# mprib/caliscope

Hardware: NVIDIA H100
Metric: lm_iterations_per_sec (higher is better)
Workload: dtype f64

## Files before the change

caliscope_b200/csrc/cb_device.cuh:

```cuda
#pragma once
#include <cuda_runtime.h>
#include <stdint.h>

namespace cb {

constexpr int CT_R = 0;
constexpr int CT_T = 9;
constexpr int CT_JR = 12;
constexpr int CT_FX = 21;
constexpr int CT_FY = 22;
constexpr int CT_CX = 23;
constexpr int CT_CY = 24;
constexpr int CT_D = 25;
constexpr int CT_IFX0 = 30;
constexpr int CT_SX = 31;
constexpr int CT_SY = 32;
constexpr int CT_FYR = 33;
constexpr int CT_FLAGS = 34;
constexpr int CT_FX0 = 35;
constexpr int CT_SIZE = 36;
constexpr int CT_SMEM = 37;

constexpr double CB_EPS = 2.220446049250313e-16;

// ... 23 lines not shown
  asm volatile("mbarrier.arrive.expect_tx.shared::cta.b64 _, [%0], %1;" ::"r"(smem_u32(bar)), "r"(bytes) : "memory");
}
__device__ __forceinline__ void mbar_wait(unsigned long long* bar, uint32_t phase) {
  asm volatile(
      "{\n"
      ".reg .pred p;\n"
      "WAIT_%=:\n"
      "mbarrier.try_wait.parity.shared::cta.b64 p, [%0], %1;\n"
      "@p bra DONE_%=;\n"
      "bra WAIT_%=;\n"
      "DONE_%=:\n"
      "}\n" ::"r"(smem_u32(bar)),
      "r"(phase)
      : "memory");
}
__device__ __forceinline__ void mbar_arrive(unsigned long long* bar) {
  asm volatile("mbarrier.arrive.shared::cta.b64 _, [%0];" ::"r"(smem_u32(bar)) : "memory");
}
__device__ __forceinline__ void bulk_g2s(void* dst_smem, const void* src_gmem, uint32_t bytes, unsigned long long* bar) {
  asm volatile("cp.async.bulk.shared::cluster.global.mbarrier::complete_tx::bytes [%0], [%1], %2, [%3];" ::"r"(
                   smem_u32(dst_smem)),
               "l"(src_gmem), "r"(bytes), "r"(smem_u32(bar))
               : "memory");
}

__device__ __forceinline__ double warp_sum(double v) {
#pragma unroll
  for (int o = 16; o > 0; o >>= 1) v += __shfl_xor_sync(0xffffffffu, v, o);
  return v;
}
__device__ __forceinline__ double warp_max(double v) {
#pragma unroll
  for (int o = 16; o > 0; o >>= 1) v = fmax(v, __shfl_xor_sync(0xffffffffu, v, o));
  return v;
}

__device__ __forceinline__ void loss_eval(int loss, double z, double& r0, double& r1, double& r2) {
  switch (loss) {
    case 1: {
      double t = 1.0 + z, s = sqrt(t);
      r0 = 2.0 * (s - 1.0);
      r1 = 1.0 / s;
      r2 = -0.5 / (t * s);
    } break;
    case 2: {
      if (z <= 1.0) {
// ... 192 lines not shown
```

caliscope_b200/csrc/cb_engine.cu:

```cuda
#include <cuda_runtime.h>
#include <dlfcn.h>
#if defined(__x86_64__)
#include <emmintrin.h>
#endif
#include <nvtx3/nvToolsExt.h>

#include <algorithm>
#include <atomic>
#include <chrono>
#include <cmath>
#include <cstdio>
#include <cstdlib>
#include <cstring>
#include <condition_variable>
#include <cub/cub.cuh>
#include <deque>
#include <functional>
#include <map>
#include <memory>
#include <mutex>
#include <string>
#include <thread>
#include <vector>

// ... 388 lines not shown
  size_t pt_smem = 0, bs_smem = 0;
  std::vector<int> h_cam_off;
  std::vector<int> h_perm, h_slot;
  std::vector<int> h_iflags;
  bool order_auto = false, order_identity = true;
  int ncp = 0;
  int *d_cam_xoff = nullptr, *d_cam_slot = nullptr, *d_klist = nullptr;
  bool schur_sparse = false;
  double schur_flop_issued = 0.0;
  std::vector<void*> allocs;
  int* d_cam_flags = nullptr;
  double* d_cam_const = nullptr;
  double2 *d_cm_xy = nullptr, *d_pm_xy = nullptr;
  int *d_cm_pt = nullptr, *d_cm_orig = nullptr, *d_cam_start = nullptr;
  int *d_chunk_cam = nullptr, *d_chunk_begin = nullptr, *d_chunk_end = nullptr, *d_cam_chunk_start = nullptr;
  int *d_pt_start = nullptr, *d_pm_orig = nullptr, *d_pm_cam = nullptr, *d_pm_pt = nullptr;
  const int *d_obs_cam = nullptr, *d_obs_pt = nullptr;
  const double* d_obs_xy = nullptr;
  std::vector<int> h_cam_flags;
  std::vector<double> h_cam_const;
  int *d_tile_of = nullptr, *d_tile_slot_start = nullptr, *d_tile_slots = nullptr;
  cb::SyItem* d_items = nullptr;
  int n_items = 0, n_slots = 0;
  unsigned char* d_active = nullptr;
  double *d_lo = nullptr, *d_hi = nullptr;
  double *d_x = nullptr, *d_xc[2] = {nullptr, nullptr}, *d_xp4[2] = {nullptr, nullptr};
  double *d_camtab[2] = {nullptr, nullptr}, *d_Upk[2] = {nullptr, nullptr}, *d_gc[2] = {nullptr, nullptr},
         *d_costsum[2] = {nullptr, nullptr};
  double *d_partial = nullptr, *d_camcost = nullptr, *d_V6 = nullptr, *d_gp = nullptr, *d_Dp2 = nullptr,
         *d_Dc2 = nullptr, *d_Linv6 = nullptr, *d_tvec = nullptr, *d_Zt = nullptr, *d_part = nullptr,
         *d_tpart = nullptr, *d_red = nullptr, *d_Minv = nullptr, *d_dc = nullptr, *d_dp = nullptr,
         *d_bpart = nullptr, *d_sc = nullptr, *d_red2 = nullptr, *d_out2 = nullptr;
  unsigned long long* d_gmax = nullptr;
  unsigned int* d_counter = nullptr;
  cb::LmState* d_state = nullptr;
  cb::LmState* h_state = nullptr;
  cb::LmLogRow* d_log = nullptr;
  int log_cap = 4096;
  double* h_x = nullptr;
  cudaEvent_t ev0 = nullptr, ev1 = nullptr, ev2 = nullptr, ev3 = nullptr, ev_state[2] = {nullptr, nullptr};
  cudaEvent_t ev_pp[2][4] = {{nullptr, nullptr, nullptr, nullptr}, {nullptr, nullptr, nullptr, nullptr}};
  cudaStream_t cap_stream = nullptr;
  TrialGraph trial_graph;
  TrialGraph loop_graph;
  int pcg_cs = 1, pcg_rows = 0, pcg_mode = 2, pcg_cl = 1, pcg_npa = 0;
  bool direct_solve = false;
// ... 319 lines not shown
  const int loss = 0;
  const double fscale = 1.0;
  launch_resjac<P, 0>(p, p->d_state, flip, loss, fscale, nullptr, st);
  if (p->n_c)
    CB_LAUNCH((cb::constraint_eval_kernel<false>), p->n_cblk, cb::CC_THREADS, 0, st, (const cb::LmState*)p->d_state, flip,
              p->ct, p->c_xp(), loss, fscale, p->m_crs(), p->m_cdirw(), (double*)nullptr, p->d_camcost + p->n_cams);
  CB_LAUNCH((cb::trial_reduce_kernel<P>), p->n_cams + 1, 64, 0, st, p->d_state, mode, p->n_cams, p->d_cam_chunk_start,
            p->d_partial, p->m_Upk(), p->m_gc(), p->m_costsum(), p->d_camcost, p->n_cblk, p->d_bpart,
            p->pt_grid + p->n_comp, p->pt_grid + p->n_comp, p->d_red2, p->d_counter, p->d_sc, p->d_log);
  return CB_OK;
}

template <int P>
int build_system(CbBaProblem* p, const CbBaOptions* opt, cudaStream_t st, const cudaEvent_t* ev = nullptr, bool cov = false) {
  if (ev) CB_CUDA(cudaEventRecord(ev[0], st));
  if (cov) launch_pt_pass<P, true>(p, st);
  else launch_pt_pass<P>(p, st);
  if (ev) CB_CUDA(cudaEventRecord(ev[1], st));
  if (p->n_c)
    CB_LAUNCH((cb::comp_build_kernel<P>), p->n_comp, cb::CC_THREADS, p->comp_build_smem, st, (const cb::LmState*)p->d_state,
              p->ct, p->d_pt_start, p->d_pm_cam, p->d_V6, p->d_gp, p->d_Dp2, p->d_gpt, p->c_crs(), p->c_cdirw(), p->n_cams,
              p->d_compL, p->d_tvec, p->d_Zt, (size_t)p->LD, p->d_gmax);
  if (ev) CB_CUDA(cudaEventRecord(ev[2], st));
  CB_LAUNCH(cb::schur_syrk_kernel, p->n_items, cb::SY_THREADS, sizeof(cb::SyrkSmem), st, (const cb::LmState*)p->d_state,
            p->d_Zt, (size_t)p->LD, p->d_tvec, p->d_items, (const int*)p->d_klist, p->d_part, p->d_tpart);
  if (ev) CB_CUDA(cudaEventRecord(ev[3], st));
  const size_t nfin = (size_t)p->nP * p->nP + p->nP + 1;
  const int rank = sharded(opt) ? std::min(std::max(opt->rank, 0), p->red_slots - 1) : 0;
  if (opt && opt->peer_group) {
    CbPeerGroup* g = (CbPeerGroup*)opt->peer_group;
    int nb = 0;
    CB_CUDA(cudaOccupancyMaxActiveBlocksPerMultiprocessor(&nb, cb::schur_finalize_peer_kernel<P>, cb::PEER_THREADS, 0));
    const int grid = std::max(1, std::min(nb, 2)) * p->num_sms;
    const cb::LmState* sd = p->d_state;
    int nP = p->nP, n_blk = p->n_blk, red_slots = p->red_slots, rk = rank;
    cb::CPtr2 upk = p->c_Upk(), gc = p->c_gc(), cs = p->c_costsum();
    const double* gmax = (const double*)p->d_gmax;
    void* args[] = {&sd, &nP, &n_blk, &p->d_tile_of, &p->d_tile_slot_start, &p->d_tile_slots, &p->d_part, &p->d_tpart,
                    &upk, &gc, &cs, &gmax, &red_slots, &rk, &g->tab, &p->d_red};
    CB_CUDA(cudaLaunchCooperativeKernel((const void*)cb::schur_finalize_peer_kernel<P>, dim3(grid), dim3(cb::PEER_THREADS),
                                        args, 0, st));
    g_launches.fetch_add(1);
  } else {
    CB_LAUNCH((cb::schur_finalize_kernel<P>), cdiv((long long)std::max<size_t>(nfin, p->red_slots), 256), 256, 0, st,
              (const cb::LmState*)p->d_state, p->nP, p->n_blk, p->d_tile_of, p->d_tile_slot_start, p->d_tile_slots,
              p->d_part, p->d_tpart, p->c_Upk(), p->c_gc(), p->c_costsum(), (const double*)p->d_gmax, p->red_slots, rank,
              p->d_red);
    if (sharded(opt)) CB_TRY(do_allreduce(opt, p->d_red, (long long)p->red_len(), st));
// ... 530 lines not shown
  switch (what) {
    case 0: return p->schur_sparse ? 1.0 : 0.0;
    case 1: return p->schur_flop_issued;
    case 2: return p->direct_solve ? 1.0 : 0.0;
    case 3: return (double)p->n_items;
    case 4: case 5: case 6: return (double)p->cov_ms[what - 4];
    case 7: return (double)p->pt_lanes;
    case 8: return p->n_dups ? 1.0 : 0.0;
    case 9: return (double)p->cam_in_smem;
    case 10: return p->direct_solve ? 0.0 : (double)p->pcg_mode;
    case 11: return (double)p->pcg_cs;
    case 12: return p->pcg_mode == 2 ? (double)p->pcg_cl : 0.0;
    case 13: return p->order_identity ? 0.0 : 1.0;
    default: return -1.0;
  }
}

static int build_schur_items(CbBaProblem* p, cudaStream_t st) {
  const int nb = p->n_blk;
  std::vector<int> tof((size_t)nb * nb, -1);
  int nt = 0;
  for (int I = 0; I < nb; ++I)
    for (int J = I; J < nb; ++J) tof[(size_t)I * nb + J] = nt++;
  const double w_pair = 1.31;
  const double w_single = 1.04;

  std::vector<long long> pair_koff, pair_cnt;
  bool sparse = false;
  int want_sparse = -1;
  if (const char* ev = std::getenv("CB_SY_SPARSE")) want_sparse = std::atoi(ev);
  if (nb >= 2 && nb <= 64 && p->n_pts > 0 && want_sparse != 0) {
    unsigned long long* d_mask;
    CB_TRY(dalloc(&d_mask, (size_t)p->n_pts));
    ScopedFree sf; sf.dev.push_back(d_mask);
    CB_LAUNCH(cb::pt_tile_mask_kernel, cdiv(p->n_pts, 256), 256, 0, st, p->d_pt_start, p->d_pm_cam, p->n_pts, p->P, d_mask);
    if (p->n_comp)
      CB_LAUNCH(cb::comp_tile_mask_kernel, cdiv(p->n_comp, 256), 256, 0, st, p->ct.comp_pt_start, p->ct.comp_pts, p->n_comp,
                d_mask);
    unsigned long long* d_cnt;
    CB_TRY(dalloc(&d_cnt, (size_t)nt));
    sf.dev.push_back(d_cnt);
    CB_CUDA(cudaMemsetAsync(d_cnt, 0, sizeof(unsigned long long) * nt, st));
    CB_LAUNCH(cb::tile_pair_count_kernel, cdiv(p->n_pts, 256), 256, sizeof(unsigned) * nt, st, d_mask, p->n_pts, nb, d_cnt);
    std::vector<unsigned long long> cnt_u((size_t)nt);
    CB_CUDA(cudaMemcpyAsync(cnt_u.data(), d_cnt, sizeof(unsigned long long) * nt, cudaMemcpyDeviceToHost, st));
    CB_CUDA(cudaStreamSynchronize(st));
    std::vector<long long> cnt(cnt_u.begin(), cnt_u.end());
    double listed = 0.0, dense = 0.0;
    for (int I = 0; I < nb; ++I)
      for (int J = I; J < nb; ++J) {
        const double w = (I == J) ? w_single : 1.0;
        listed += w * (double)cnt[tof[(size_t)I * nb + J]];
        dense += w * (double)p->n_pts;
      }
    sparse = want_sparse == 1 || listed < 0.7 * dense;
    if (sparse) {
      const int zero_row = p->K_pad;
      std::vector<long long> pair_start((size_t)nt + 1, 0), koff_h((size_t)nt, -1);
      long long klen = 0;
      for (int t = 0; t < nt; ++t) {
        pair_start[(size_t)t + 1] = pair_start[(size_t)t] + cnt[(size_t)t];
        if (cnt[(size_t)t] == 0) continue;
        koff_h[(size_t)t] = klen;
        klen += cdiv(3 * cnt[(size_t)t], (long long)cb::SY_KC) * cb::SY_KC;
      }
      const long long n_inc = pair_start[(size_t)nt];
      if (klen > 0x7fffffffLL || n_inc > 0x7fffffffLL) { g_last_error = "Schur row lists exceed 2^31 entries"; return CB_E_UNSUPPORTED; }
      pair_koff.assign(koff_h.begin(), koff_h.end());
      pair_cnt.assign(cnt.begin(), cnt.end());
      int *d_ninc = nullptr, *d_incoff = nullptr;
      unsigned long long *d_keys = nullptr, *d_keys_s = nullptr;
      long long *d_pair_start = nullptr, *d_koff = nullptr;
      CB_TRY(dalloc(&d_ninc, (size_t)p->n_pts + 1)); sf.dev.push_back(d_ninc);
      CB_TRY(dalloc(&d_incoff, (size_t)p->n_pts + 1)); sf.dev.push_back(d_incoff);
// ... 23 lines not shown
      CB_LAUNCH(cb::klist_expand_kernel, cdiv(n_inc, 256), 256, 0, st, (const unsigned long long*)d_keys_s, n_inc, p->n_pts,
                (const long long*)d_pair_start, (const long long*)d_koff, p->d_klist);
      CB_CUDA(cudaStreamSynchronize(st));
    }
  }
  p->schur_sparse = sparse;

  struct Group { int kind, I, J; double w; int chunks; int koff; };
  std::vector<Group> groups;
  if (!sparse) {
    for (int I = 0; I < nb; ++I)
      for (int J = I + 1; J < nb; ++J) groups.push_back({0, I, J, 1.0, p->k_chunks, -1});
    for (int I = 0; I < nb; I += 2) {
      if (I + 1 < nb) groups.push_back({1, I, I + 1, w_pair, p->k_chunks, -1});
      else groups.push_back({1, I, -1, w_single, p->k_chunks, -1});
    }
  } else {
    for (int I = 0; I < nb; ++I)
      for (int J = I; J < nb; ++J) {
        const int t = tof[(size_t)I * nb + J];
        if (pair_cnt[(size_t)t] == 0) continue;
        const int koff = (int)pair_koff[(size_t)t];
        const int chunks = (int)cdiv(3 * pair_cnt[(size_t)t], (long long)cb::SY_KC);
        if (I == J) groups.push_back({1, I, -1, w_single, chunks, koff});
        else groups.push_back({0, I, J, 1.0, chunks, koff});
      }
  }
  double W = 0.0;
  for (auto& g : groups) W += g.w * g.chunks;
  p->schur_flop_issued = 0.0;
  for (auto& g : groups) {
    const double cols2 = g.kind == 0 ? 96.0 * 96.0 : (g.J >= 0 ? 2.0 : 1.0) * 42.0 * 16.0 * 8.0;
    p->schur_flop_issued += 2.0 * cols2 * (double)g.chunks * cb::SY_KC;
  }
  std::vector<cb::SyItem> items;
  std::vector<std::vector<int>> slots_of(nt);
  int slot = 0;
  constexpr int SY_MIN_CHUNKS = 8;
  auto cap_of = [&](const Group& g) { return std::max(1, g.chunks / SY_MIN_CHUNKS); };
  std::vector<int> n_of(groups.size(), 1);
  {
    int used = 0;
    for (size_t gi = 0; gi < groups.size(); ++gi) {
      const Group& g = groups[gi];
      int n = (int)std::floor(p->num_sms * (g.w * g.chunks) / std::max(W, 1.0));
      n_of[gi] = std::max(1, std::min(n, cap_of(g)));
      used += n_of[gi];
// ... 301 lines not shown
  for (int c = 0; c < p->n_cams; ++c)
    for (int a = 0; a < ((p->h_iflags[c] & CB_CAM_FREE_INTRINSICS) ? 9 : 6); ++a) act[(size_t)c * p->P + a] = 1;
  CB_TRY(palloc(p, &p->d_active, p->nP));
  CB_CUDA(cudaMemcpyAsync(p->d_active, act.data(), p->nP, cudaMemcpyHostToDevice, st));
  CB_CUDA(cudaStreamSynchronize(st));
  CB_TRY(palloc(p, &p->d_lo, p->nP)); CB_TRY(palloc(p, &p->d_hi, p->nP));

  const int NACC = (p->P == 6) ? 28 : 55, NU = (p->P == 6) ? 21 : 45;
  const size_t npts = (size_t)std::max(p->n_pts, 1);
  CB_TRY(palloc(p, &p->d_x, (size_t)p->n_params + 1));
  for (int k = 0; k < 2; ++k) {
    CB_TRY(palloc(p, &p->d_xc[k], p->nP)); CB_TRY(palloc(p, &p->d_xp4[k], 4 * npts));
    CB_TRY(palloc(p, &p->d_camtab[k], (size_t)p->n_cams * cb::CT_SIZE));
    CB_TRY(palloc(p, &p->d_Upk[k], (size_t)p->n_cams * NU)); CB_TRY(palloc(p, &p->d_gc[k], p->nP));
    CB_TRY(palloc(p, &p->d_costsum[k], 4));
  }
  CB_TRY(palloc(p, &p->d_partial, (size_t)std::max(p->n_chunks, 1) * NACC + p->n_cblk));
  CB_TRY(palloc(p, &p->d_camcost, (size_t)p->n_cams + p->n_cblk));
  CB_TRY(palloc(p, &p->d_gpt, 3 * npts));
  CB_TRY(palloc(p, &p->d_V6, 6 * npts)); CB_TRY(palloc(p, &p->d_gp, 3 * npts)); CB_TRY(palloc(p, &p->d_Dp2, 3 * npts));
  CB_TRY(palloc(p, &p->d_Dc2, p->nP)); CB_TRY(palloc(p, &p->d_Linv6, 6 * npts));
  CB_TRY(palloc(p, &p->d_tvec, (size_t)p->K_pad + cb::SY_KC));
  CB_TRY(palloc(p, &p->d_Zt, ((size_t)p->K_pad + cb::SY_KC) * p->LD));
  CB_TRY(palloc(p, &p->d_part, (size_t)p->n_slots * cb::SY_TILE * cb::SY_TILE));
  CB_TRY(palloc(p, &p->d_tpart, (size_t)p->n_slots * cb::SY_TILE));
  CB_TRY(palloc(p, &p->d_red, p->red_len()));
  CB_TRY(palloc(p, &p->d_Minv, (size_t)p->n_cams * p->P * p->P));
  CB_TRY(palloc(p, &p->d_dc, p->nP)); CB_TRY(palloc(p, &p->d_dp, 3 * npts));
  CB_TRY(palloc(p, &p->d_bpart, 3 * ((size_t)p->pt_grid + p->n_comp)));
  CB_TRY(palloc(p, &p->d_sc, cb::SC_COUNT)); CB_TRY(palloc(p, &p->d_red2, 8));
  CB_TRY(palloc(p, &p->d_gmax, 2));
  CB_TRY(palloc(p, &p->d_counter, 4));
  CB_TRY(palloc(p, &p->d_state, 1));
  CB_TRY(palloc(p, &p->d_log, (size_t)p->log_cap));
  CB_TRY(palloc(p, &p->d_out2, 2 * (size_t)std::max(n, 1)));
  CB_CUDA(cudaMemsetAsync(p->d_Zt, 0, sizeof(double) * ((size_t)p->K_pad + cb::SY_KC) * p->LD, st));
  CB_CUDA(cudaMemsetAsync(p->d_tvec, 0, sizeof(double) * ((size_t)p->K_pad + cb::SY_KC), st));
  CB_CUDA(cudaMemsetAsync(p->d_tpart, 0, sizeof(double) * (size_t)p->n_slots * cb::SY_TILE, st));
  CB_CUDA(cudaMemsetAsync(p->d_part, 0, sizeof(double) * (size_t)p->n_slots * cb::SY_TILE * cb::SY_TILE, st));
  CB_CUDA(cudaMemsetAsync(p->d_red2, 0, sizeof(double) * 8, st));
  CB_CUDA(cudaMemsetAsync(p->d_Linv6, 0, sizeof(double) * 6 * npts, st));
  CB_TRY(cached_malloc_host((void**)&p->h_state, sizeof(cb::LmState) * 4));
  CB_TRY(cached_malloc_host((void**)&p->h_x, sizeof(double) * ((size_t)p->n_params + 1)));
  for (cudaEvent_t* e : {&p->ev0, &p->ev1, &p->ev2, &p->ev3, &p->ev_pp[0][0], &p->ev_pp[0][1], &p->ev_pp[0][2], &p->ev_pp[0][3],
                         &p->ev_pp[1][0], &p->ev_pp[1][1], &p->ev_pp[1][2], &p->ev_pp[1][3]})
    CB_CUDA(cudaEventCreate(e));
// ... 1824 lines not shown
```

caliscope_b200/csrc/cb_kernels.cuh:

```cuda
#pragma once
#include <cooperative_groups.h>

#include "cb_device.cuh"

namespace cb {
namespace cg = cooperative_groups;

constexpr int RJ_THREADS = 128;
constexpr int RJ_CHUNK = 2048;
constexpr int PT_WARPS = 8;
constexpr int SY_TILE = 96;
constexpr int SY_KC = 32;
constexpr int SY_STAGES = 4;
constexpr int SY_CONSUMER_WARPS = 8;
constexpr int SY_THREADS = 32 * (SY_CONSUMER_WARPS + 1);
constexpr int PCG_THREADS = 512;

template <int P>
struct RowT {
  static constexpr int NU = P * (P + 1) / 2;
  static constexpr int NACC = NU + P + 1;
};

enum {
// ... 245 lines not shown
  const double e00 = V6[0] + lam * d0, e01 = V6[1], e02 = V6[2], e11 = V6[3] + lam * d1, e12 = V6[4],
               e22 = V6[5] + lam * d2;
  bool ok = e00 > 0.0;
  const double i00 = rsqrt(ok ? e00 : 1.0);
  const double l10 = e01 * i00, l20 = e02 * i00;
  const double t11 = e11 - l10 * l10;
  ok = ok && t11 > 0.0;
  const double i11 = rsqrt(ok ? t11 : 1.0);
  const double l21 = (e12 - l20 * l10) * i11;
  const double t22 = e22 - l20 * l20 - l21 * l21;
  ok = ok && t22 > 0.0;
  const double i22 = rsqrt(ok ? t22 : 1.0);
  const double i10 = -l10 * i00 * i11;
  const double i21 = -l21 * i11 * i22;
  const double i20 = -(l20 * i00 + l21 * i10) * i22;
  if (ok) {
    Li[0] = i00; Li[1] = i10; Li[2] = i11; Li[3] = i20; Li[4] = i21; Li[5] = i22;
  } else {
    Li[0] = Li[1] = Li[2] = Li[3] = Li[4] = Li[5] = 0.0;
  }
}

constexpr int SY_LDS = SY_TILE + 4;

struct SyrkSmem {
  double A[SY_STAGES][SY_KC * SY_LDS];
  double B[SY_STAGES][SY_KC * SY_LDS];
  double t[SY_STAGES][SY_KC];
  unsigned long long full[SY_STAGES];
  unsigned long long empty[SY_STAGES];
};

__device__ __forceinline__ void dmma884(double& c0, double& c1, double a, double b) {
  asm volatile("mma.sync.aligned.m8n8k4.row.col.f64.f64.f64.f64 {%0,%1}, {%2}, {%3}, {%0,%1};"
               : "+d"(c0), "+d"(c1)
               : "d"(a), "d"(b));
}

__device__ __forceinline__ void dmma16816(double (&c)[4], const double (&a)[8], const double (&b)[4]) {
  asm("mma.sync.aligned.m16n8k16.row.col.f64.f64.f64.f64 {%0,%1,%2,%3}, {%4,%5,%6,%7,%8,%9,%10,%11}, {%12,%13,%14,%15}, "
      "{%0,%1,%2,%3};"
      : "+d"(c[0]), "+d"(c[1]), "+d"(c[2]), "+d"(c[3])
      : "d"(a[0]), "d"(a[1]), "d"(a[2]), "d"(a[3]), "d"(a[4]), "d"(a[5]), "d"(a[6]), "d"(a[7]), "d"(b[0]), "d"(b[1]),
        "d"(b[2]), "d"(b[3]));
}

// ... 55 lines not shown
#pragma unroll
      for (int j0 = 0; j0 < SY_DIAG_MAX; j0 += BATCH) {
        if (j0 + BATCH <= lo || j0 >= hi) continue;
        double b[BATCH][4];
#pragma unroll
        for (int jj = 0; jj < BATCH; ++jj) {
          const int j = j0 + jj;
          if (j < SY_DIAG_MAX && j >= lo && j < hi) {
#pragma unroll
            for (int q = 0; q < 4; ++q) b[jj][q] = Tk[4 * q * SY_LDS + (c0 + j) * 8];
          }
        }
#pragma unroll
        for (int jj = 0; jj < BATCH; ++jj) {
          const int j = j0 + jj;
          if (j < SY_DIAG_MAX && j >= lo && j < hi) dmma16816(acc[j], a, b[jj]);
        }
      }
    }
  }
}

__global__ void __launch_bounds__(SY_THREADS, 1)
schur_syrk_kernel(const LmState* __restrict__ st, const double* __restrict__ Zt, size_t LD,
                  const double* __restrict__ tvec, const SyItem* __restrict__ items, const int* __restrict__ klist,
                  double* __restrict__ part, double* __restrict__ tpart) {
  extern __shared__ __align__(128) unsigned char smem_raw[];
  SyrkSmem& sm = *reinterpret_cast<SyrkSmem*>(smem_raw);
  if (st->done) return;
  const SyItem item = items[blockIdx.x];
  const bool diag = item.kind == 1;
  const bool two = diag ? (item.J >= 0) : true;
  const int tid = threadIdx.x, lane = tid & 31, wid = tid >> 5;
  const int fr = lane >> 2, fk = lane & 3;

  if (tid == 0) {
    for (int s = 0; s < SY_STAGES; ++s) {
      mbar_init(&sm.full[s], 1);
      mbar_init(&sm.empty[s], SY_CONSUMER_WARPS);
    }
    mbar_fence_init();
  }
  __syncthreads();

  const uint32_t row_bytes = SY_TILE * 8;
  const uint32_t stage_bytes = SY_KC * row_bytes * (two ? 2u : 1u);
  const int n_it = item.c1 - item.c0;

  if (wid == SY_CONSUMER_WARPS) {
    for (int it = 0; it < n_it; ++it) {
      const int stage = it % SY_STAGES, round = it / SY_STAGES;
      if (round > 0) mbar_wait(&sm.empty[stage], (uint32_t)((round - 1) & 1));
      const size_t k = item.koff >= 0 ? (size_t)klist[(size_t)item.koff + (size_t)(item.c0 + it) * SY_KC + lane]
                                      : (size_t)(item.c0 + it) * SY_KC + lane;
      if (diag) sm.t[stage][lane] = tvec[k];
      __syncwarp();
      if (lane == 0) mbar_expect_tx(&sm.full[stage], stage_bytes);
      __syncwarp();
      bulk_g2s(&sm.A[stage][lane * SY_LDS], Zt + k * LD + (size_t)item.I * SY_TILE, row_bytes, &sm.full[stage]);
      if (two)
        bulk_g2s(&sm.B[stage][lane * SY_LDS], Zt + k * LD + (size_t)item.J * SY_TILE, row_bytes, &sm.full[stage]);
    }
    return;
  }

  if (!diag) {
    const int wr = wid >> 2, wc = wid & 3;
    double acc[3][3][4];
#pragma unroll
    for (int u = 0; u < 3; ++u)
#pragma unroll
      for (int v = 0; v < 3; ++v)
#pragma unroll
        for (int e = 0; e < 4; ++e) acc[u][v][e] = 0.0;
    for (int it = 0; it < n_it; ++it) {
      const int stage = it % SY_STAGES;
      mbar_wait(&sm.full[stage], (uint32_t)((it / SY_STAGES) & 1));
      syrk_offdiag_stage(acc, sm.A[stage], sm.B[stage], wr, wc, fr, fk);
      __syncwarp();
// ... 24 lines not shown
    const int stage = it % SY_STAGES;
    mbar_wait(&sm.full[stage], (uint32_t)((it / SY_STAGES) & 1));
    syrk_diag_stage(acc, run.sel == 0 ? sm.A[stage] : sm.B[stage], run, fr, fk);
    if (tact) {
      const double* Ad = (tsel == 0 ? sm.A[stage] : sm.B[stage]);
#pragma unroll 8
      for (int k = 0; k < SY_KC; ++k) tacc = fma(Ad[k * SY_LDS + trow], sm.t[stage][k], tacc);
    }
    __syncwarp();
    if (lane == 0) mbar_arrive(&sm.empty[stage]);
  }
  double* out = part + (size_t)(run.sel == 0 ? item.slotA : item.slotB) * (SY_TILE * SY_TILE);
#pragma unroll
  for (int j = 0; j < SY_DIAG_MAX; ++j) {
    if (j >= nA + nB) break;
    const int rb = j < nA ? rA : rB, cb = j < nA ? cA + j : cB + (j - nA);
#pragma unroll
    for (int h = 0; h < 2; ++h) {
      const int r = rb * 16 + 8 * h + fr, cc = cb * 8 + 2 * fk;
      *reinterpret_cast<double2*>(out + r * SY_TILE + cc) = make_double2(acc[j][2 * h], acc[j][2 * h + 1]);
    }
  }
  if (tact) tpart[(size_t)(tsel == 0 ? item.slotA : item.slotB) * SY_TILE + trow] = tacc;
}

template <int P>
__device__ __forceinline__ void finalize_elem(size_t idx, int nP, int n_blk, const int* __restrict__ tile_of,
                                              const int* __restrict__ tile_slot_start,
                                              const int* __restrict__ tile_slots, const double* __restrict__ part,
                                              const double* __restrict__ tpart, const double* __restrict__ Upk,
                                              const double* __restrict__ gc, const double* __restrict__ cam_cost_sum,
                                              double* __restrict__ red) {
  using RT = RowT<P>;
  const size_t nn = (size_t)nP * nP;
  if (idx < nn) {
    const int i = (int)(idx / nP), j = (int)(idx % nP);
    int I = i / SY_TILE, J = j / SY_TILE, li = i % SY_TILE, lj = j % SY_TILE;
    if (I > J) { int t = I; I = J; J = t; t = li; li = lj; lj = t; }
    if (I == J && li > lj) { int t = li; li = lj; lj = t; }
    const int tile = tile_of[I * n_blk + J];
    double s = 0.0;
    const int q1 = tile_slot_start[tile + 1];
#pragma unroll 8
    for (int q = tile_slot_start[tile]; q < q1; ++q)
      s += part[(size_t)tile_slots[q] * (SY_TILE * SY_TILE) + li * SY_TILE + lj];
    double u = 0.0;
// ... 594 lines not shown
```

profiles/microbench/syrk_feed.cu:

```cuda
#include <algorithm>
#include <cmath>
#include <cstdio>
#include <vector>

#include "../../caliscope_b200/csrc/cb_kernels.cuh"

using cb::bulk_g2s;
using cb::mbar_arrive;
using cb::mbar_expect_tx;
using cb::mbar_fence_init;
using cb::mbar_init;
using cb::mbar_wait;

constexpr int TILE = 96, LDS = TILE + 4, NB = 4, LD = NB * TILE, N_PTS = 50000;
constexpr int STAGES = 4, CWARPS = 8, THREADS = 32 * (CWARPS + 1);

__device__ __forceinline__ void dmma884(double& c0, double& c1, double a, double b) {
  asm volatile("mma.sync.aligned.m8n8k4.row.col.f64.f64.f64.f64 {%0,%1}, {%2}, {%3}, {%0,%1};"
               : "+d"(c0), "+d"(c1) : "d"(a), "d"(b));
}
__device__ __forceinline__ void dmma16816(double (&c)[4], const double (&a)[8], const double (&b)[4]) {
  asm volatile("mma.sync.aligned.m16n8k16.row.col.f64.f64.f64.f64 {%0,%1,%2,%3}, {%4,%5,%6,%7,%8,%9,%10,%11}, "
               "{%12,%13,%14,%15}, {%0,%1,%2,%3};"
               : "+d"(c[0]), "+d"(c[1]), "+d"(c[2]), "+d"(c[3])
// ... 94 lines not shown
#pragma unroll
            for (int u = 0; u < 3; ++u) a[u] = T[br * 24 + u * 8];
#pragma unroll
            for (int v = 0; v < 3; ++v) bb[v] = T[bc * 24 + v * 8];
#pragma unroll
            for (int u = 0; u < 3; ++u)
#pragma unroll
              for (int v = 0; v < 3; ++v) dmma884(acc[b][u][v][0], acc[b][u][v][1], a[u], bb[v]);
          }
      }
      __syncwarp();
      if (MODE != 2 && lane == 0) mbar_arrive(&sm.empty[stage]);
    }
#pragma unroll
    for (int b = 0; b < 3; ++b)
#pragma unroll
      for (int u = 0; u < 3; ++u)
#pragma unroll
        for (int v = 0; v < 3; ++v) sum += acc[b][u][v][0] + acc[b][u][v][1];
  }
  out[(size_t)blockIdx.x * THREADS + tid] = sum;
}

template <int MODE>
__global__ void __launch_bounds__(cb::SY_THREADS, 1) engine_feed(const double* __restrict__ Zt,
                                                                const cb::SyItem* __restrict__ items,
                                                                double* __restrict__ out) {
  extern __shared__ __align__(128) unsigned char raw[];
  cb::SyrkSmem& sm = *reinterpret_cast<cb::SyrkSmem*>(raw);
  const cb::SyItem item = items[blockIdx.x];
  const bool diag = item.kind == 1, two = diag ? item.J >= 0 : true;
  const int tid = threadIdx.x, lane = tid & 31, wid = tid >> 5, fr = lane >> 2, fk = lane & 3;
  if (tid == 0) {
    for (int s = 0; s < cb::SY_STAGES; ++s) { mbar_init(&sm.full[s], 1); mbar_init(&sm.empty[s], cb::SY_CONSUMER_WARPS); }
    mbar_fence_init();
  }
  __syncthreads();
  const int n_it = item.c1 - item.c0;
  const uint32_t row_bytes = TILE * 8;
  if (wid == cb::SY_CONSUMER_WARPS) {
    if constexpr (MODE != 2) {
      for (int it = 0; it < n_it; ++it) {
        const int stage = it % cb::SY_STAGES, round = it / cb::SY_STAGES;
        if (round > 0) mbar_wait(&sm.empty[stage], (uint32_t)((round - 1) & 1));
        const size_t k = (size_t)(item.c0 + it) * cb::SY_KC + lane;
        if (lane == 0) mbar_expect_tx(&sm.full[stage], cb::SY_KC * row_bytes * (two ? 2u : 1u));
        __syncwarp();
        bulk_g2s(&sm.A[stage][lane * LDS], Zt + k * LD + (size_t)item.I * TILE, row_bytes, &sm.full[stage]);
        if (two) bulk_g2s(&sm.B[stage][lane * LDS], Zt + k * LD + (size_t)item.J * TILE, row_bytes, &sm.full[stage]);
      }
    }
    return;
  }
  double sum = 0.0;
  if (!diag) {
    double acc[3][3][4] = {};
    for (int it = 0; it < n_it; ++it) {
      const int stage = it % cb::SY_STAGES;
      if (MODE != 2) mbar_wait(&sm.full[stage], (uint32_t)((it / cb::SY_STAGES) & 1));
      if (MODE != 1) cb::syrk_offdiag_stage(acc, sm.A[stage], sm.B[stage], wid >> 2, wid & 3, fr, fk);
      __syncwarp();
      if (MODE != 2 && lane == 0) mbar_arrive(&sm.empty[stage]);
    }
    for (int u = 0; u < 3; ++u)
      for (int v = 0; v < 3; ++v) sum += acc[u][v][0] + acc[u][v][1] + acc[u][v][2] + acc[u][v][3];
  } else {
    const cb::SyDiagRuns run = cb::SY_DIAG_RUNS[two ? 0 : 1][wid];
    double acc[cb::SY_DIAG_MAX][4] = {};
    for (int it = 0; it < n_it; ++it) {
      const int stage = it % cb::SY_STAGES;
      if (MODE != 2) mbar_wait(&sm.full[stage], (uint32_t)((it / cb::SY_STAGES) & 1));
      if (MODE != 1) cb::syrk_diag_stage(acc, run.sel == 0 ? sm.A[stage] : sm.B[stage], run, fr, fk);
// ... 96 lines not shown
           bytes, 0.0);
    report("(c) MMA on resident stages, no loads", time_ms([&] { old_feed<2><<<grid, THREADS, smem>>>(Zt, d_items, out); }, reps),
           0.0, flop);
    std::vector<Item> off(sms, Item{0, 0, 1, 0, 256}), pair(sms, Item{1, 0, 1, 0, 256});
    Item* d_w;
    cudaMalloc(&d_w, sms * sizeof(Item));
    cudaMemcpy(d_w, off.data(), sms * sizeof(Item), cudaMemcpyHostToDevice);
    const float t_off = time_ms([&] { old_feed<2><<<sms, THREADS, smem>>>(Zt, d_w, out); }, reps);
    cudaMemcpy(d_w, pair.data(), sms * sizeof(Item), cudaMemcpyHostToDevice);
    const float t_pair = time_ms([&] { old_feed<2><<<sms, THREADS, smem>>>(Zt, d_w, out); }, reps);
    printf("per-item feed: diagonal pair / off-diagonal CTA cost (MMA only) = %.3f\n", t_pair / t_off);
    printf("feed bytes per launch: %.3f GB\n", bytes * 1e-9);
    cudaFree(d_w);
    cudaFree(d_items);
  }
  {
    cb::LmState h_st{};
    cb::LmState* d_st;
    cudaMalloc(&d_st, sizeof(cb::LmState));
    cudaMemcpy(d_st, &h_st, sizeof(cb::LmState), cudaMemcpyHostToDevice);
    double *part, *tpart;
    cudaMalloc(&part, (size_t)2 * sms * TILE * TILE * sizeof(double));
    cudaMalloc(&tpart, (size_t)2 * sms * TILE * sizeof(double));
    const int smem = sizeof(cb::SyrkSmem);
    cudaFuncSetAttribute(cb::schur_syrk_kernel, cudaFuncAttributeMaxDynamicSharedMemorySize, smem);
    cb::SyItem* d_it;
    cudaMalloc(&d_it, 2 * sms * sizeof(cb::SyItem));
    auto run = [&](const std::vector<cb::SyItem>& v) {
      cudaMemcpy(d_it, v.data(), v.size() * sizeof(cb::SyItem), cudaMemcpyHostToDevice);
      return time_ms([&] {
        cb::schur_syrk_kernel<<<(int)v.size(), cb::SY_THREADS, smem>>>(d_st, Zt, LD, Zt, d_it, nullptr, part, tpart);
      }, reps);
    };
    auto mk = [&](int kind, int I, int J, int c0, int c1, int s) { return cb::SyItem{kind, I, J, c0, c1, s, s + sms, -1}; };
    const int ch = 256;
    std::vector<cb::SyItem> off, pair, single;
    for (int s = 0; s < sms; ++s) {
      off.push_back(mk(0, 0, 1, 0, ch, s));
      pair.push_back(mk(1, 0, 1, 0, ch, s));
      single.push_back(mk(1, 0, -1, 0, ch, s));
    }
    const float t_off = run(off), t_pair = run(pair), t_single = run(single);
    const double fl_off = 2.0 * 96 * 96 * ch * KC_OLD * sms;
    report("(e) engine kernel, off-diagonal CTAs only", t_off, 2.0 * ch * KC_OLD * TILE * 8 * sms, fl_off);
    report("(e) engine kernel, diagonal-pair CTAs only", t_pair, 2.0 * ch * KC_OLD * TILE * 8 * sms, fl_off * 84 / 72);
    report("(e) engine kernel, single-diagonal CTAs only", t_single, 1.0 * ch * KC_OLD * TILE * 8 * sms, fl_off * 42 / 72);
    printf("engine kernel: diagonal pair / off-diagonal = %.3f, single diagonal / off-diagonal = %.3f\n", t_pair / t_off,
           t_single / t_off);
    const std::vector<Item> sched = old_items(sms, K_pad / KC_OLD, t_pair / t_off);
    std::vector<cb::SyItem> v;
    double bytes = 0.0, flop = 0.0;
    for (size_t i = 0; i < sched.size(); ++i) {
      const Item& x = sched[i];
      v.push_back(mk(x.kind, x.I, x.J, x.c0, x.c1, (int)i));
      bytes += 2.0 * (x.c1 - x.c0) * KC_OLD * TILE * 8;
      flop += 2.0 * (x.kind == 0 ? 96.0 * 96.0 : 84.0 * 16 * 8) * (x.c1 - x.c0) * KC_OLD;
    }
    report("(e) engine kernel, cfg4 schedule at the measured weight", run(v), bytes, flop);
    cudaFuncSetAttribute(engine_feed<0>, cudaFuncAttributeMaxDynamicSharedMemorySize, smem);
    cudaFuncSetAttribute(engine_feed<1>, cudaFuncAttributeMaxDynamicSharedMemorySize, smem);
    cudaFuncSetAttribute(engine_feed<2>, cudaFuncAttributeMaxDynamicSharedMemorySize, smem);
    auto run_mode = [&](int mode, const std::vector<cb::SyItem>& items) {
      cudaMemcpy(d_it, items.data(), items.size() * sizeof(cb::SyItem), cudaMemcpyHostToDevice);
      const int g = (int)items.size();
      return time_ms([&] {
        if (mode == 0) engine_feed<0><<<g, cb::SY_THREADS, smem>>>(Zt, d_it, out);
        else if (mode == 1) engine_feed<1><<<g, cb::SY_THREADS, smem>>>(Zt, d_it, out);
        else engine_feed<2><<<g, cb::SY_THREADS, smem>>>(Zt, d_it, out);
      }, reps);
    };
    report("(d) engine math, cfg4 schedule, loads + MMA", run_mode(0, v), bytes, flop);
    report("(d) engine math, cfg4 schedule, loads only", run_mode(1, v), bytes, 0.0);
    report("(d) engine math, cfg4 schedule, MMA only", run_mode(2, v), 0.0, flop);
    const float m_off = run_mode(2, off), m_pair = run_mode(2, pair), m_single = run_mode(2, single);
    report("(d) engine math, off-diagonal CTAs only, MMA only", m_off, 0.0, fl_off);
    report("(d) engine math, diagonal-pair CTAs only, MMA only", m_pair, 0.0, fl_off * 84 / 72);
    report("(d) engine math, single-diagonal CTAs only, MMA only", m_single, 0.0, fl_off * 42 / 72);
    cudaFree(d_it); cudaFree(part); cudaFree(tpart); cudaFree(d_st);
  }
  cudaFree(Zt);
  cudaFree(out);
  return 0;
}
```

Before: 794.7.

## Load dense Schur SYRK stages with 2D TMA tensor boxes and retune diagonal weights

For dense (non-listed) SYRK items, the producer warp now issues a single 2D tensor-map TMA load per operand per stage instead of 32 per-row bulk copies, removing per-lane copy issue overhead. The box is SY_LDS wide, so padded columns are also transferred, which adds some bandwidth. The scheduler's diagonal-pair and single-diagonal cost weights are raised for dense scheduling, while listed scheduling keeps the old single weight, changing load balance across CTAs. A tensor map is encoded at setup through the driver entry point, and the microbenchmark gains box and lock-step variants.

```diff
diff --git a/caliscope_b200/csrc/cb_device.cuh b/caliscope_b200/csrc/cb_device.cuh
--- a/caliscope_b200/csrc/cb_device.cuh
+++ b/caliscope_b200/csrc/cb_device.cuh
@@ -1,4 +1,5 @@
 #pragma once
+#include <cuda.h>
 #include <cuda_runtime.h>
 #include <stdint.h>
 
@@ -69,6 +70,13 @@
                    smem_u32(dst_smem)),
                "l"(src_gmem), "r"(bytes), "r"(smem_u32(bar))
                : "memory");
+}
+__device__ __forceinline__ void tma_load_2d(void* dst_smem, const CUtensorMap* map, int c0, int c1, unsigned long long* bar) {
+  asm volatile(
+      "cp.async.bulk.tensor.2d.shared::cluster.global.mbarrier::complete_tx::bytes [%0], [%1, {%2, %3}], [%4];" ::"r"(
+          smem_u32(dst_smem)),
+      "l"(reinterpret_cast<uint64_t>(map)), "r"(c0), "r"(c1), "r"(smem_u32(bar))
+      : "memory");
 }
 
 __device__ __forceinline__ double warp_sum(double v) {
diff --git a/caliscope_b200/csrc/cb_engine.cu b/caliscope_b200/csrc/cb_engine.cu
--- a/caliscope_b200/csrc/cb_engine.cu
+++ b/caliscope_b200/csrc/cb_engine.cu
@@ -434,6 +434,7 @@
   int *d_tile_of = nullptr, *d_tile_slot_start = nullptr, *d_tile_slots = nullptr;
   cb::SyItem* d_items = nullptr;
   int n_items = 0, n_slots = 0;
+  CUtensorMap zt_map{};
   unsigned char* d_active = nullptr;
   double *d_lo = nullptr, *d_hi = nullptr;
   double *d_x = nullptr, *d_xc[2] = {nullptr, nullptr}, *d_xp4[2] = {nullptr, nullptr};
@@ -799,8 +800,9 @@
               p->ct, p->d_pt_start, p->d_pm_cam, p->d_V6, p->d_gp, p->d_Dp2, p->d_gpt, p->c_crs(), p->c_cdirw(), p->n_cams,
               p->d_compL, p->d_tvec, p->d_Zt, (size_t)p->LD, p->d_gmax);
   if (ev) CB_CUDA(cudaEventRecord(ev[2], st));
-  CB_LAUNCH(cb::schur_syrk_kernel, p->n_items, cb::SY_THREADS, sizeof(cb::SyrkSmem), st, (const cb::LmState*)p->d_state,
-            p->d_Zt, (size_t)p->LD, p->d_tvec, p->d_items, (const int*)p->d_klist, p->d_part, p->d_tpart);
+  CB_LAUNCH(cb::schur_syrk_kernel, p->n_items, cb::SY_THREADS, sizeof(cb::SyrkSmem), st, p->zt_map,
+            (const cb::LmState*)p->d_state, p->d_Zt, (size_t)p->LD, p->d_tvec, p->d_items, (const int*)p->d_klist,
+            p->d_part, p->d_tpart);
   if (ev) CB_CUDA(cudaEventRecord(ev[3], st));
   const size_t nfin = (size_t)p->nP * p->nP + p->nP + 1;
   const int rank = sharded(opt) ? std::min(std::max(opt->rank, 0), p->red_slots - 1) : 0;
@@ -1377,8 +1379,9 @@
   int nt = 0;
   for (int I = 0; I < nb; ++I)
     for (int J = I; J < nb; ++J) tof[(size_t)I * nb + J] = nt++;
-  const double w_pair = 1.31;
-  const double w_single = 1.04;
+  const double w_pair = 2.07;
+  const double w_single = 1.46;
+  const double w_list_single = 1.04;
 
   std::vector<long long> pair_koff, pair_cnt;
   bool sparse = false;
@@ -1404,7 +1407,7 @@
     double listed = 0.0, dense = 0.0;
     for (int I = 0; I < nb; ++I)
       for (int J = I; J < nb; ++J) {
-        const double w = (I == J) ? w_single : 1.0;
+        const double w = (I == J) ? w_list_single : 1.0;
         listed += w * (double)cnt[tof[(size_t)I * nb + J]];
         dense += w * (double)p->n_pts;
       }
@@ -1474,7 +1477,7 @@
         if (pair_cnt[(size_t)t] == 0) continue;
         const int koff = (int)pair_koff[(size_t)t];
         const int chunks = (int)cdiv(3 * pair_cnt[(size_t)t], (long long)cb::SY_KC);
-        if (I == J) groups.push_back({1, I, -1, w_single, chunks, koff});
+        if (I == J) groups.push_back({1, I, -1, w_list_single, chunks, koff});
         else groups.push_back({0, I, J, 1.0, chunks, koff});
       }
   }
@@ -1822,6 +1825,7 @@
   CB_TRY(palloc(p, &p->d_Dc2, p->nP)); CB_TRY(palloc(p, &p->d_Linv6, 6 * npts));
   CB_TRY(palloc(p, &p->d_tvec, (size_t)p->K_pad + cb::SY_KC));
   CB_TRY(palloc(p, &p->d_Zt, ((size_t)p->K_pad + cb::SY_KC) * p->LD));
+  CB_CUDA(cb::make_zt_tensor_map(&p->zt_map, p->d_Zt, (size_t)p->LD, (size_t)p->K_pad + cb::SY_KC));
   CB_TRY(palloc(p, &p->d_part, (size_t)p->n_slots * cb::SY_TILE * cb::SY_TILE));
   CB_TRY(palloc(p, &p->d_tpart, (size_t)p->n_slots * cb::SY_TILE));
   CB_TRY(palloc(p, &p->d_red, p->red_len()));
diff --git a/caliscope_b200/csrc/cb_kernels.cuh b/caliscope_b200/csrc/cb_kernels.cuh
--- a/caliscope_b200/csrc/cb_kernels.cuh
+++ b/caliscope_b200/csrc/cb_kernels.cuh
@@ -291,6 +291,7 @@
 }
 
 constexpr int SY_LDS = SY_TILE + 4;
+static_assert(SY_KC * SY_LDS * sizeof(double) % 128 == 0, "Schur stage size");
 
 struct SyrkSmem {
   double A[SY_STAGES][SY_KC * SY_LDS];
@@ -392,9 +393,10 @@
 }
 
 __global__ void __launch_bounds__(SY_THREADS, 1)
-schur_syrk_kernel(const LmState* __restrict__ st, const double* __restrict__ Zt, size_t LD,
-                  const double* __restrict__ tvec, const SyItem* __restrict__ items, const int* __restrict__ klist,
-                  double* __restrict__ part, double* __restrict__ tpart) {
+schur_syrk_kernel(const __grid_constant__ CUtensorMap zt_map, const LmState* __restrict__ st,
+                  const double* __restrict__ Zt, size_t LD, const double* __restrict__ tvec,
+                  const SyItem* __restrict__ items, const int* __restrict__ klist, double* __restrict__ part,
+                  double* __restrict__ tpart) {
   extern __shared__ __align__(128) unsigned char smem_raw[];
   SyrkSmem& sm = *reinterpret_cast<SyrkSmem*>(smem_raw);
   if (st->done) return;
@@ -414,17 +416,26 @@
   __syncthreads();
 
   const uint32_t row_bytes = SY_TILE * 8;
-  const uint32_t stage_bytes = SY_KC * row_bytes * (two ? 2u : 1u);
+  const bool listed = item.koff >= 0;
+  const uint32_t stage_bytes = SY_KC * (listed ? row_bytes : SY_LDS * 8u) * (two ? 2u : 1u);
   const int n_it = item.c1 - item.c0;
 
   if (wid == SY_CONSUMER_WARPS) {
     for (int it = 0; it < n_it; ++it) {
-      const int stage = it % SY_STAGES, round = it / SY_STAGES;
+      const int stage = it % SY_STAGES, round = it / SY_STAGES, chunk = item.c0 + it;
       if (round > 0) mbar_wait(&sm.empty[stage], (uint32_t)((round - 1) & 1));
-      const size_t k = item.koff >= 0 ? (size_t)klist[(size_t)item.koff + (size_t)(item.c0 + it) * SY_KC + lane]
-                                      : (size_t)(item.c0 + it) * SY_KC + lane;
+      const size_t k = listed ? (size_t)klist[(size_t)item.koff + (size_t)chunk * SY_KC + lane]
+                              : (size_t)chunk * SY_KC + lane;
       if (diag) sm.t[stage][lane] = tvec[k];
       __syncwarp();
+      if (!listed) {
+        if (lane == 0) {
+          mbar_expect_tx(&sm.full[stage], stage_bytes);
+          tma_load_2d(sm.A[stage], &zt_map, item.I * SY_TILE, chunk * SY_KC, &sm.full[stage]);
+          if (two) tma_load_2d(sm.B[stage], &zt_map, item.J * SY_TILE, chunk * SY_KC, &sm.full[stage]);
+        }
+        continue;
+      }
       if (lane == 0) mbar_expect_tx(&sm.full[stage], stage_bytes);
       __syncwarp();
       bulk_g2s(&sm.A[stage][lane * SY_LDS], Zt + k * LD + (size_t)item.I * SY_TILE, row_bytes, &sm.full[stage]);
@@ -495,6 +506,23 @@
     }
   }
   if (tact) tpart[(size_t)(tsel == 0 ? item.slotA : item.slotB) * SY_TILE + trow] = tacc;
+}
+
+inline cudaError_t make_zt_tensor_map(CUtensorMap* map, const double* Zt, size_t ld, size_t rows) {
+  using Encode = CUresult (*)(CUtensorMap*, CUtensorMapDataType, cuuint32_t, void*, const cuuint64_t*, const cuuint64_t*,
+                              const cuuint32_t*, const cuuint32_t*, CUtensorMapInterleave, CUtensorMapSwizzle,
+                              CUtensorMapL2promotion, CUtensorMapFloatOOBfill);
+  void* fn = nullptr;
+  cudaDriverEntryPointQueryResult q = cudaDriverEntryPointSymbolNotFound;
+  const cudaError_t e = cudaGetDriverEntryPoint("cuTensorMapEncodeTiled", &fn, cudaEnableDefault, &q);
+  if (e != cudaSuccess) return e;
+  if (q != cudaDriverEntryPointSuccess || !fn) return cudaErrorSymbolNotFound;
+  const cuuint64_t dim[2] = {ld, rows}, stride[1] = {ld * sizeof(double)};
+  const cuuint32_t box[2] = {SY_LDS, SY_KC}, estride[2] = {1, 1};
+  const CUresult r = ((Encode)fn)(map, CU_TENSOR_MAP_DATA_TYPE_FLOAT64, 2, const_cast<double*>(Zt), dim, stride, box,
+                                  estride, CU_TENSOR_MAP_INTERLEAVE_NONE, CU_TENSOR_MAP_SWIZZLE_NONE,
+                                  CU_TENSOR_MAP_L2_PROMOTION_L2_256B, CU_TENSOR_MAP_FLOAT_OOB_FILL_NONE);
+  return r == CUDA_SUCCESS ? cudaSuccess : cudaErrorInvalidValue;
 }
 
 template <int P>
diff --git a/profiles/microbench/syrk_feed.cu b/profiles/microbench/syrk_feed.cu
--- a/profiles/microbench/syrk_feed.cu
+++ b/profiles/microbench/syrk_feed.cu
@@ -140,9 +140,11 @@
   out[(size_t)blockIdx.x * THREADS + tid] = sum;
 }
 
-template <int MODE>
-__global__ void __launch_bounds__(cb::SY_THREADS, 1) engine_feed(const double* __restrict__ Zt,
+template <int MODE, bool BOX = false>
+__global__ void __launch_bounds__(cb::SY_THREADS, 1) engine_feed(const __grid_constant__ CUtensorMap zt_map,
+                                                                const double* __restrict__ Zt,
                                                                 const cb::SyItem* __restrict__ items,
+                                                                const int* __restrict__ cstep,
                                                                 double* __restrict__ out) {
   extern __shared__ __align__(128) unsigned char raw[];
   cb::SyrkSmem& sm = *reinterpret_cast<cb::SyrkSmem*>(raw);
@@ -154,18 +156,26 @@
     mbar_fence_init();
   }
   __syncthreads();
-  const int n_it = item.c1 - item.c0;
+  const int step = cstep[blockIdx.x], n_it = (item.c1 - item.c0 + step - 1) / step;
   const uint32_t row_bytes = TILE * 8;
   if (wid == cb::SY_CONSUMER_WARPS) {
     if constexpr (MODE != 2) {
       for (int it = 0; it < n_it; ++it) {
-        const int stage = it % cb::SY_STAGES, round = it / cb::SY_STAGES;
+        const int stage = it % cb::SY_STAGES, round = it / cb::SY_STAGES, chunk = item.c0 + it * step;
         if (round > 0) mbar_wait(&sm.empty[stage], (uint32_t)((round - 1) & 1));
-        const size_t k = (size_t)(item.c0 + it) * cb::SY_KC + lane;
-        if (lane == 0) mbar_expect_tx(&sm.full[stage], cb::SY_KC * row_bytes * (two ? 2u : 1u));
-        __syncwarp();
-        bulk_g2s(&sm.A[stage][lane * LDS], Zt + k * LD + (size_t)item.I * TILE, row_bytes, &sm.full[stage]);
-        if (two) bulk_g2s(&sm.B[stage][lane * LDS], Zt + k * LD + (size_t)item.J * TILE, row_bytes, &sm.full[stage]);
+        if constexpr (BOX) {
+          if (lane == 0) {
+            mbar_expect_tx(&sm.full[stage], cb::SY_KC * LDS * 8 * (two ? 2u : 1u));
+            cb::tma_load_2d(sm.A[stage], &zt_map, item.I * TILE, chunk * cb::SY_KC, &sm.full[stage]);
+            if (two) cb::tma_load_2d(sm.B[stage], &zt_map, item.J * TILE, chunk * cb::SY_KC, &sm.full[stage]);
+          }
+        } else {
+          const size_t k = (size_t)chunk * cb::SY_KC + lane;
+          if (lane == 0) mbar_expect_tx(&sm.full[stage], cb::SY_KC * row_bytes * (two ? 2u : 1u));
+          __syncwarp();
+          bulk_g2s(&sm.A[stage][lane * LDS], Zt + k * LD + (size_t)item.I * TILE, row_bytes, &sm.full[stage]);
+          if (two) bulk_g2s(&sm.B[stage][lane * LDS], Zt + k * LD + (size_t)item.J * TILE, row_bytes, &sm.full[stage]);
+        }
       }
     }
     return;
@@ -308,6 +318,11 @@
     double *part, *tpart;
     cudaMalloc(&part, (size_t)2 * sms * TILE * TILE * sizeof(double));
     cudaMalloc(&tpart, (size_t)2 * sms * TILE * sizeof(double));
+    CUtensorMap zmap;
+    if (cb::make_zt_tensor_map(&zmap, Zt, LD, (size_t)K_pad + KC_OLD) != cudaSuccess) {
+      printf("tensor map encoding failed\n");
+      return 1;
+    }
     const int smem = sizeof(cb::SyrkSmem);
     cudaFuncSetAttribute(cb::schur_syrk_kernel, cudaFuncAttributeMaxDynamicSharedMemorySize, smem);
     cb::SyItem* d_it;
@@ -315,7 +330,7 @@
     auto run = [&](const std::vector<cb::SyItem>& v) {
       cudaMemcpy(d_it, v.data(), v.size() * sizeof(cb::SyItem), cudaMemcpyHostToDevice);
       return time_ms([&] {
-        cb::schur_syrk_kernel<<<(int)v.size(), cb::SY_THREADS, smem>>>(d_st, Zt, LD, Zt, d_it, nullptr, part, tpart);
+        cb::schur_syrk_kernel<<<(int)v.size(), cb::SY_THREADS, smem>>>(zmap, d_st, Zt, LD, Zt, d_it, nullptr, part, tpart);
       }, reps);
     };
     auto mk = [&](int kind, int I, int J, int c0, int c1, int s) { return cb::SyItem{kind, I, J, c0, c1, s, s + sms, -1}; };
@@ -333,36 +348,72 @@
     report("(e) engine kernel, single-diagonal CTAs only", t_single, 1.0 * ch * KC_OLD * TILE * 8 * sms, fl_off * 42 / 72);
     printf("engine kernel: diagonal pair / off-diagonal = %.3f, single diagonal / off-diagonal = %.3f\n", t_pair / t_off,
            t_single / t_off);
-    const std::vector<Item> sched = old_items(sms, K_pad / KC_OLD, t_pair / t_off);
-    std::vector<cb::SyItem> v;
     double bytes = 0.0, flop = 0.0;
-    for (size_t i = 0; i < sched.size(); ++i) {
-      const Item& x = sched[i];
-      v.push_back(mk(x.kind, x.I, x.J, x.c0, x.c1, (int)i));
-      bytes += 2.0 * (x.c1 - x.c0) * KC_OLD * TILE * 8;
-      flop += 2.0 * (x.kind == 0 ? 96.0 * 96.0 : 84.0 * 16 * 8) * (x.c1 - x.c0) * KC_OLD;
-    }
+    std::vector<int> steps;
+    auto sched = [&](double w, bool lockstep) {
+      const std::vector<Item> g = old_items(sms, K_pad / KC_OLD, w);
+      std::vector<cb::SyItem> v;
+      steps.clear();
+      bytes = flop = 0.0;
+      for (size_t i = 0; i < g.size();) {
+        size_t e = i;
+        while (e < g.size() && g[e].kind == g[i].kind && g[e].I == g[i].I && g[e].J == g[i].J) ++e;
+        const int n = (int)(e - i);
+        for (size_t q = i; q < e; ++q) {
+          const Item& x = g[q];
+          v.push_back(lockstep ? mk(x.kind, x.I, x.J, (int)(q - i), K_pad / KC_OLD, (int)q)
+                               : mk(x.kind, x.I, x.J, x.c0, x.c1, (int)q));
+          steps.push_back(lockstep ? n : 1);
+          bytes += 2.0 * (x.c1 - x.c0) * KC_OLD * TILE * 8;
+          flop += 2.0 * (x.kind == 0 ? 96.0 * 96.0 : 84.0 * 16 * 8) * (x.c1 - x.c0) * KC_OLD;
+        }
+        i = e;
+      }
+      return v;
+    };
+    report("(e) engine kernel, cfg4 schedule at w_pair 1.31", run(sched(1.31, false)), bytes, flop);
+    const std::vector<cb::SyItem> vl = sched(t_pair / t_off, true);
+    const std::vector<int> steps_l = steps;
+    const std::vector<cb::SyItem> v = sched(t_pair / t_off, false);
     report("(e) engine kernel, cfg4 schedule at the measured weight", run(v), bytes, flop);
     cudaFuncSetAttribute(engine_feed<0>, cudaFuncAttributeMaxDynamicSharedMemorySize, smem);
     cudaFuncSetAttribute(engine_feed<1>, cudaFuncAttributeMaxDynamicSharedMemorySize, smem);
     cudaFuncSetAttribute(engine_feed<2>, cudaFuncAttributeMaxDynamicSharedMemorySize, smem);
-    auto run_mode = [&](int mode, const std::vector<cb::SyItem>& items) {
+    cudaFuncSetAttribute(engine_feed<0, true>, cudaFuncAttributeMaxDynamicSharedMemorySize, smem);
+    cudaFuncSetAttribute(engine_feed<1, true>, cudaFuncAttributeMaxDynamicSharedMemorySize, smem);
+    int* d_step;
+    cudaMalloc(&d_step, 2 * sms * sizeof(int));
+    auto run_mode = [&](int mode, const std::vector<cb::SyItem>& items, const std::vector<int>* st = nullptr) {
+      const std::vector<int> ones(items.size(), 1);
       cudaMemcpy(d_it, items.data(), items.size() * sizeof(cb::SyItem), cudaMemcpyHostToDevice);
+      cudaMemcpy(d_step, (st ? *st : ones).data(), items.size() * sizeof(int), cudaMemcpyHostToDevice);
       const int g = (int)items.size();
       return time_ms([&] {
-        if (mode == 0) engine_feed<0><<<g, cb::SY_THREADS, smem>>>(Zt, d_it, out);
-        else if (mode == 1) engine_feed<1><<<g, cb::SY_THREADS, smem>>>(Zt, d_it, out);
-        else engine_feed<2><<<g, cb::SY_THREADS, smem>>>(Zt, d_it, out);
+        if (mode == 0) engine_feed<0><<<g, cb::SY_THREADS, smem>>>(zmap, Zt, d_it, d_step, out);
+        else if (mode == 1) engine_feed<1><<<g, cb::SY_THREADS, smem>>>(zmap, Zt, d_it, d_step, out);
+        else if (mode == 2) engine_feed<2><<<g, cb::SY_THREADS, smem>>>(zmap, Zt, d_it, d_step, out);
+        else if (mode == 3) engine_feed<0, true><<<g, cb::SY_THREADS, smem>>>(zmap, Zt, d_it, d_step, out);
+        else engine_feed<1, true><<<g, cb::SY_THREADS, smem>>>(zmap, Zt, d_it, d_step, out);
       }, reps);
     };
-    report("(d) engine math, cfg4 schedule, loads + MMA", run_mode(0, v), bytes, flop);
-    report("(d) engine math, cfg4 schedule, loads only", run_mode(1, v), bytes, 0.0);
+    report("(d) engine math, cfg4 schedule, loads + MMA (row copies)", run_mode(0, v), bytes, flop);
+    report("(d) engine math, cfg4 schedule, loads + MMA (boxes)", run_mode(3, v), bytes, flop);
+    report("(d) engine math, lock-step schedule, loads + MMA (row copies)", run_mode(0, vl, &steps_l), bytes, flop);
+    report("(d) engine math, lock-step schedule, loads + MMA (boxes)", run_mode(3, vl, &steps_l), bytes, flop);
+    report("(d)(i) loads only, row copies", run_mode(1, v), bytes, 0.0);
+    report("(d)(ii) loads only, tensor boxes", run_mode(4, v), bytes, 0.0);
+    report("(d)(iii) loads only, row copies, lock-step", run_mode(1, vl, &steps_l), bytes, 0.0);
+    report("(d)(ii+iii) loads only, tensor boxes, lock-step", run_mode(4, vl, &steps_l), bytes, 0.0);
     report("(d) engine math, cfg4 schedule, MMA only", run_mode(2, v), 0.0, flop);
     const float m_off = run_mode(2, off), m_pair = run_mode(2, pair), m_single = run_mode(2, single);
     report("(d) engine math, off-diagonal CTAs only, MMA only", m_off, 0.0, fl_off);
     report("(d) engine math, diagonal-pair CTAs only, MMA only", m_pair, 0.0, fl_off * 84 / 72);
     report("(d) engine math, single-diagonal CTAs only, MMA only", m_single, 0.0, fl_off * 42 / 72);
-    cudaFree(d_it); cudaFree(part); cudaFree(tpart); cudaFree(d_st);
+    printf("engine math, MMA only: diagonal pair / off-diagonal = %.3f, single diagonal / off-diagonal = %.3f\n",
+           m_pair / m_off, m_single / m_off);
+    const std::vector<cb::SyItem> vm = sched(m_pair / m_off, false);
+    report("(d) engine math, schedule at the MMA-only weight, MMA only", run_mode(2, vm), 0.0, flop);
+    cudaFree(d_step); cudaFree(d_it); cudaFree(part); cudaFree(tpart); cudaFree(d_st);
   }
   cudaFree(Zt);
   cudaFree(out);
```

Measured after the change: 872.6, median of 6. +9.8%, better.
